# jfkirk/tensorrec

Measured on AMD Instinct MI355X. Metric: user-item predictions/sec, higher is better.
Workload: dtype i8/bf16/fp32; 1 GPU; synthetic 1000000 users x 1000000 items, identity features, d=128, LinearRepresentation + DotProduct, biased, fused top-10 (BASELINE.json configs[2]); users=1000000, items=1000000, n_components=128, top_k=10, parallelism=items sharded x1, users replicated, topk_method=two_stage

## Files before the change

### tensorrec_amd/csrc/score_blockmax_i8.hip

```cpp
#include "score_common.hpp"
#include <math.h>
#include <limits.h>
#include <type_traits>

namespace {

typedef int v4i32 __attribute__((ext_vector_type(4)));
typedef int v16i32 __attribute__((ext_vector_type(16)));

constexpr int BNQ = 128;

template <int KT, bool BIAS, int NCB, int WPS, int TK>
__global__ __launch_bounds__(256, WPS) void blockmax_i8_kernel(ScoreParams p)
{
    constexpr int RB = KT;
    constexpr int CH = RB / 16;
    constexpr int KS = KT / 32;
    constexpr int TILE_BYTES = BNQ * RB;
    constexpr int NSLOT = BNQ * CH / 256;
    constexpr int NBLK = BNQ / 32;
    constexpr int NSTEP = NBLK * KS;
    static_assert(KT == 64 || KT == 128 || KT == 256, "int8 BLOCKMAX covers K = 64 / 128 / 256");

    extern __shared__ __attribute__((aligned(16))) char smem[];
    int* side = (int*)(smem + 2 * TILE_BYTES);

    const int tid = threadIdx.x;
    const int lane = tid & 63;
    const int wave = __builtin_amdgcn_readfirstlane(tid >> 6);
    const int half = lane >> 5, l31 = lane & 31;
    const int rblock = blockIdx.x % p.n_rblocks;
    const int chunk = blockIdx.x / p.n_rblocks;
    const int64_t r_base = ((int64_t)rblock * 4 + wave) * (NCB * 32);
    const int64_t t_begin = (int64_t)chunk * p.chunk_len;
    const int64_t t_end = (t_begin + p.chunk_len < p.n_t) ? t_begin + p.chunk_len : p.n_t;
    const int n_tiles = (int)((t_end - t_begin + BNQ - 1) / BNQ);

    v4i32 rfq[NCB][KS];
    float r_bias[NCB];
#pragma unroll
    for (int cb = 0; cb < NCB; ++cb) {
        int64_t row = r_base + cb * 32 + l31;
        if (row >= p.n_r) row = p.n_r - 1;
        const char* src = (const char*)p.R + row * (int64_t)RB;
#pragma unroll
        for (int ks = 0; ks < KS; ++ks) rfq[cb][ks] = *(const v4i32*)(src + (ks * 2 + half) * 16);
        r_bias[cb] = (BIAS && p.r_bias) ? p.r_bias[row] : 0.f;
    }

    int slot_off[NSLOT];
#pragma unroll
    for (int i = 0; i < NSLOT; ++i) {
        const int q = i * 256 + tid;
        const int row = q / CH, pc = q % CH;
        const int sw = CH >= 16 ? (row & 15) : (CH == 8 ? ((row >> 1) & 7) : ((row >> 2) & 3));
        slot_off[i] = row * RB + ((pc ^ sw) * 16);
    }
    const char* t_chunk = (const char*)p.T + t_begin * (int64_t)RB;
    const int* t_bias_q = p.t_bias ? (const int*)p.t_bias + (p.wg_class ? (int64_t)p.wg_class[rblock] * p.bias_stride : 0) : nullptr;
    auto stage_issue = [&](int tile, int buf) {
        const int64_t row0 = t_begin + (int64_t)tile * BNQ;
        const bool clamp = row0 + BNQ > p.n_t;
        if (BIAS && wave < 2) {
            int64_t g = row0 + wave * 64 + lane;
            if (g >= p.n_t) g = p.n_t - 1;
            if (t_bias_q) {
                __builtin_amdgcn_global_load_lds((const __attribute__((address_space(1))) void*)(t_bias_q + g),
                                                 (__attribute__((address_space(3))) void*)(side + buf * BNQ + wave * 64), 4, 0, 0);
            } else {
                side[buf * BNQ + wave * 64 + lane] = 0;
            }
        }
        const char* tile_base = t_chunk + (int64_t)tile * (BNQ * RB);
#pragma unroll
        for (int i = 0; i < NSLOT; ++i) {
            int off = slot_off[i];
            if (clamp) {
                const int last = (int)(p.n_t - 1 - row0);
                const int row = (i * 256 + tid) / CH;
                if (row > last) off -= (row - last) * RB;
            }
            char* dst = smem + buf * TILE_BYTES + (i * 256 + wave * 64) * 16;
            __builtin_amdgcn_global_load_lds((const __attribute__((address_space(1))) void*)(tile_base + off),
                                             (__attribute__((address_space(3))) void*)dst, 16, 0, 0);
        }
    };

    int koff[KS];
    {
        const int sw = CH >= 16 ? (l31 & 15) : (CH == 8 ? ((l31 >> 1) & 7) : ((l31 >> 2) & 3));
#pragma unroll
        for (int ks = 0; ks < KS; ++ks) koff[ks] = l31 * RB + (((ks * 2 + half) ^ sw) * 16);
    }

    v16i32 acc[NCB];
    int bm[NCB];
#pragma unroll
    for (int cb = 0; cb < NCB; ++cb) bm[cb] = INT_MIN;
    float top[TK ? NCB : 1][TK ? TK : 1];
    float e_nx[TK ? NCB : 1], e_ex[TK ? NCB : 1], e_cu[TK ? NCB : 1];
    if (TK) {
#pragma unroll
        for (int cb = 0; cb < NCB; ++cb) {
            int64_t row = r_base + cb * 32 + l31;
            if (row >= p.n_r) row = p.n_r - 1;
            e_nx[cb] = p.r_err[row * 4]; e_ex[cb] = p.r_err[row * 4 + 1]; e_cu[cb] = p.r_err[row * 4 + 2];
#pragma unroll
            for (int j = 0; j < TK; ++j) top[cb][j] = -INFINITY;
        }
    }

    auto read_c0 = [&](v16i32& c, const int* sdi) {
#pragma unroll
        for (int q = 0; q < 4; ++q) {
            const v4i32 tb4 = *(const v4i32*)(sdi + 8 * q);
            c[4 * q] = tb4[0]; c[4 * q + 1] = tb4[1]; c[4 * q + 2] = tb4[2]; c[4 * q + 3] = tb4[3];
        }
    };

    auto tile_body = [&](auto bufc) __attribute__((always_inline)) {
        constexpr int buf = decltype(bufc)::value;
        const char* tb = smem + buf * TILE_BYTES;
        const int* sd = side + buf * BNQ + 4 * half;
        v4i32 tf[3];
        if (BIAS) read_c0(acc[0], sd);
        tf[0] = *(const v4i32*)(tb + koff[0]);
        tf[1] = *(const v4i32*)(tb + (KS > 1 ? koff[1 % KS] : 32 * RB + koff[0]));
        __builtin_amdgcn_sched_barrier(0);
#pragma unroll
        for (int s = 0; s < NSTEP; ++s) {
            const int blk = s / KS, ks = s % KS;
            if (s + 2 < NSTEP)
                tf[(s + 2) % 3] = *(const v4i32*)(tb + ((s + 2) / KS) * 32 * RB + koff[(s + 2) % KS]);
            if (ks == 0) {
                if (BIAS) {
#pragma unroll
                    for (int cb = NCB - 1; cb >= 0; --cb)
                        acc[cb] = __builtin_amdgcn_mfma_i32_32x32x32_i8(tf[s % 3], rfq[cb][0], acc[0], 0, 0, 0);
                } else {
                    const v16i32 z = {0, 0, 0, 0, 0, 0, 0, 0, 0, 0, 0, 0, 0, 0, 0, 0};
#pragma unroll
                    for (int cb = 0; cb < NCB; ++cb)
                        acc[cb] = __builtin_amdgcn_mfma_i32_32x32x32_i8(tf[s % 3], rfq[cb][0], z, 0, 0, 0);
                }
            } else {
#pragma unroll
                for (int cb = 0; cb < NCB; ++cb)
                    acc[cb] = __builtin_amdgcn_mfma_i32_32x32x32_i8(tf[s % 3], rfq[cb][ks], acc[cb], 0, 0, 0);
            }
            if (ks == KS - 1) {
#pragma unroll
                for (int j = 0; j < 8; ++j) bm[0] = max(max(bm[0], acc[0][2 * j]), acc[0][2 * j + 1]);
                if (BIAS && blk + 1 < NBLK) read_c0(acc[0], sd + 32 * (blk + 1));
#pragma unroll
                for (int j = 0; j < 8; ++j)
#pragma unroll
                    for (int cb = 1; cb < NCB; ++cb) bm[cb] = max(max(bm[cb], acc[cb][2 * j]), acc[cb][2 * j + 1]);
            }
            __builtin_amdgcn_sched_barrier(0);
        }
    };

    stage_issue(0, 0);
    asm volatile("s_waitcnt vmcnt(0)" ::: "memory");
    __syncthreads();

    const float a_user = p.wg_scale ? p.wg_scale[rblock] : p.scales[0];
    const int64_t sb0 = t_begin / ((int64_t)p.sb_tiles * BNQ);
    f32x4 ss_cur = *(const f32x4*)(p.sb_stats + sb0 * 4), ss_next = ss_cur;
    for (int t = 0; t < n_tiles; ++t) {
        const int buf = t & 1;
        if (t + 1 < n_tiles) stage_issue(t + 1, buf ^ 1);
        if ((t % p.sb_tiles) == 0 && t + p.sb_tiles < n_tiles)
            ss_next = *(const f32x4*)(p.sb_stats + (sb0 + t / p.sb_tiles + 1) * 4);
        if (buf == 0) tile_body(std::integral_constant<int, 0>{});
        else tile_body(std::integral_constant<int, 1>{});

        if (((t + 1) % p.sb_tiles) == 0 || t + 1 == n_tiles) {
            const int64_t sb = sb0 + t / p.sb_tiles;
            const float scale = a_user * ss_cur[0];
            const float yh = TK ? ss_cur[1] : 0.f, dy = TK ? ss_cur[2] : 0.f, db = TK ? a_user * ss_cur[3] : 0.f;
            ss_cur = ss_next;
#pragma unroll
            for (int cb = 0; cb < NCB; ++cb) {
                const int o = __shfl_xor(bm[cb], 32, 64);
                const int m = bm[cb] > o ? bm[cb] : o;
                float v = (float)m * scale;
                if (BIAS) v = v + r_bias[cb];
                const int64_t u = r_base + cb * 32 + l31;
                if (half == 0 && u < p.n_r) p.blockmax[sb * p.bm_stride + u] = v;
                bm[cb] = INT_MIN;
                if (TK) {
                    float lb = v - i8_pair_err(e_nx[cb], e_ex[cb], e_cu[cb], yh, dy, db, KT);
                    lb = (lb == lb) ? lb : -INFINITY;
                    if (p.top_tag) lb = lb_tag(lb, t / p.sb_tiles);
#pragma unroll
                    for (int j = TK - 1; j >= 1; --j) top[cb][j] = __builtin_amdgcn_fmed3f(top[cb][j], top[cb][j - 1], lb);
                    top[cb][0] = fmaxf(top[cb][0], lb);
                }
            }
        }
        if (t + 1 < n_tiles) asm volatile("s_waitcnt vmcnt(0)" ::: "memory");
        __syncthreads();
    }
    if (TK) {
#pragma unroll
        for (int cb = 0; cb < NCB; ++cb) {
            const int64_t u = r_base + cb * 32 + l31;
            if (half == 0 && u < p.n_r) {
#pragma unroll
                for (int j = 0; j < TK; ++j) p.chunk_top[((int64_t)chunk * TK + j) * p.bm_stride + u] = top[cb][j];
            }
        }
    }
}

template <int KT, bool BIAS, int TK, int NUB, int NW, int BT, int RDL = 1>
__global__ __launch_bounds__(NW * 64, 8 / NW) void blockmax_i8x16_kernel(ScoreParams p)
{
    constexpr int NT = NW * 64;
    constexpr int OW = NUB / 4;
    static_assert(NUB % 4 == 0, "user blocks per wave must split over the four row-groups");
    constexpr int RB = KT;
    constexpr int CH = RB / 16;
    constexpr int KS = KT / 64;
    constexpr int TILE_BYTES = BT * RB;
    constexpr int NSLOT = BT * CH / NT;
    constexpr int NBLK = BT / 16;
    constexpr int NSTEP = NBLK * KS;
    static_assert(KT == 64 || KT == 128, "int8 16x16x64 BLOCKMAX covers K = 64 / 128");

    extern __shared__ __attribute__((aligned(16))) char smem[];
    int* side = (int*)(smem + 2 * TILE_BYTES);

    const int tid = threadIdx.x;
    const int lane = tid & 63;
    const int wave = __builtin_amdgcn_readfirstlane(tid >> 6);
    const int g = lane >> 4, lu = lane & 15;
    const int rblock = blockIdx.x % p.n_rblocks;
    const int chunk = blockIdx.x / p.n_rblocks;
    if (p.wg_scale && p.wg_scale[rblock] == 0.f) return;
    const int64_t r_base = ((int64_t)rblock * NW + wave) * (NUB * 16);
    const int64_t t_begin = (int64_t)chunk * p.chunk_len;
    const int64_t t_end = (t_begin + p.chunk_len < p.n_t) ? t_begin + p.chunk_len : p.n_t;
    const int n_tiles = (int)((t_end - t_begin + BT - 1) / BT);
    auto swz = [](int row) { return CH == 8 ? (row & 7) : ((row >> 1) & 3); };

    v4i32 rfq[NUB][KS];
#pragma unroll
    for (int ub = 0; ub < NUB; ++ub) {
        int64_t row = r_base + ub * 16 + lu;
        if (row >= p.n_r) row = p.n_r - 1;
        const char* src = (const char*)p.R + row * (int64_t)RB;
#pragma unroll
        for (int ks = 0; ks < KS; ++ks) rfq[ub][ks] = *(const v4i32*)(src + (ks * 4 + g) * 16);
    }
    int64_t own_u[OW];
    float own_bias[OW], e_nx[OW], e_ex[OW], e_cu[OW];
    float top[TK ? OW : 1][TK ? TK : 1];
#pragma unroll
    for (int o = 0; o < OW; ++o) {
        own_u[o] = r_base + (OW * g + o) * 16 + lu;
        const int64_t row = own_u[o] < p.n_r ? own_u[o] : p.n_r - 1;
        own_bias[o] = (BIAS && p.r_bias) ? p.r_bias[row] : 0.f;
        if (TK) {
            e_nx[o] = p.r_err[row * 4]; e_ex[o] = p.r_err[row * 4 + 1]; e_cu[o] = p.r_err[row * 4 + 2];
#pragma unroll
            for (int j = 0; j < TK; ++j) top[o][j] = -INFINITY;
        }
    }

    int slot_off[NSLOT];
#pragma unroll
    for (int i = 0; i < NSLOT; ++i) {
        const int q = i * NT + tid;
        const int row = q / CH, pc = q % CH;
        slot_off[i] = row * RB + ((pc ^ swz(row)) * 16);
    }
    const char* t_chunk = (const char*)p.T + t_begin * (int64_t)RB;
    const int* t_bias_q = p.t_bias ? (const int*)p.t_bias + (p.wg_class ? (int64_t)p.wg_class[rblock] * p.bias_stride : 0) : nullptr;
    auto stage_issue = [&](int tile, int buf) {
        const int64_t row0 = t_begin + (int64_t)tile * BT;
        const bool clamp = row0 + BT > p.n_t;
        if (BIAS && wave < BT / 64) {
            int64_t gi = row0 + wave * 64 + lane;
            if (gi >= p.n_t) gi = p.n_t - 1;
            if (t_bias_q) {
                __builtin_amdgcn_global_load_lds((const __attribute__((address_space(1))) void*)(t_bias_q + gi),
                                                 (__attribute__((address_space(3))) void*)(side + buf * BT + wave * 64), 4, 0, 0);
            } else {
                side[buf * BT + wave * 64 + lane] = 0;
            }
        }
        const char* tile_base = t_chunk + (int64_t)tile * (BT * RB);
#pragma unroll
        for (int i = 0; i < NSLOT; ++i) {
            int off = slot_off[i];
            if (clamp) {
                const int last = (int)(p.n_t - 1 - row0);
                const int row = (i * NT + tid) / CH;
                if (row > last) off -= (row - last) * RB;
            }
            char* dst = smem + buf * TILE_BYTES + (i * NT + wave * 64) * 16;
            __builtin_amdgcn_global_load_lds((const __attribute__((address_space(1))) void*)(tile_base + off),
                                             (__attribute__((address_space(3))) void*)dst, 16, 0, 0);
        }
    };

    int koff[KS];
#pragma unroll
    for (int ks = 0; ks < KS; ++ks) koff[ks] = lu * RB + (((ks * 4 + g) ^ swz(lu)) * 16);

    v4i32 acc[NUB];
    int bm[NUB];
#pragma unroll
    for (int ub = 0; ub < NUB; ++ub) bm[ub] = INT_MIN;

    auto tile_body = [&](auto bufc) __attribute__((always_inline)) {
        constexpr int buf = decltype(bufc)::value;
        const char* tb = smem + buf * TILE_BYTES;
        const int* sd = side + buf * BT + 4 * g;
        v4i32 tf[3];
        v4i32 c0 = {0, 0, 0, 0};
        if (BIAS) c0 = *(const v4i32*)sd;
        tf[0] = *(const v4i32*)(tb + koff[0]);
        tf[1] = *(const v4i32*)(tb + (KS > 1 ? koff[1 % KS] : 16 * RB + koff[0]));
        __builtin_amdgcn_sched_barrier(0);
#pragma unroll
        for (int s = 0; s < NSTEP; ++s) {
            const int blk = s / KS, ks = s % KS;
            auto prefetch = [&]() {
                if (s + 2 < NSTEP) tf[(s + 2) % 3] = *(const v4i32*)(tb + ((s + 2) / KS) * 16 * RB + koff[(s + 2) % KS]);
            };
            if (RDL == 0) prefetch();
            if (ks == 0) {
#pragma unroll
                for (int ub = 0; ub < NUB; ++ub) {
                    acc[ub] = __builtin_amdgcn_mfma_i32_16x16x64_i8(tf[s % 3], rfq[ub][0], c0, 0, 0, 0);
                    if (RDL == 2 && ub == NUB / 2 - 1) { __builtin_amdgcn_sched_barrier(0); prefetch(); __builtin_amdgcn_sched_barrier(0); }
                }
                if (RDL == 1) __builtin_amdgcn_sched_barrier(0);
                if (BIAS && blk + 1 < NBLK) c0 = *(const v4i32*)(sd + 16 * (blk + 1));
            } else {
#pragma unroll
                for (int ub = 0; ub < NUB; ++ub) {
                    acc[ub] = __builtin_amdgcn_mfma_i32_16x16x64_i8(tf[s % 3], rfq[ub][ks], acc[ub], 0, 0, 0);
                    if (RDL == 2 && ub == NUB / 2 - 1) { __builtin_amdgcn_sched_barrier(0); prefetch(); __builtin_amdgcn_sched_barrier(0); }
                }
                if (RDL == 1) __builtin_amdgcn_sched_barrier(0);
            }
            if (RDL == 1 || RDL == 3) prefetch();
            if (ks == KS - 1) {
#pragma unroll
                for (int ub = 0; ub < NUB; ++ub) {
                    bm[ub] = max(max(bm[ub], acc[ub][0]), acc[ub][1]);
                    bm[ub] = max(max(bm[ub], acc[ub][2]), acc[ub][3]);
                }
            }
            if (RDL == 3) {
                if (ks == KS - 1) {
                    __builtin_amdgcn_sched_group_barrier(0x008, 3, 0);
#pragma unroll
                    for (int i = 0; i < NUB - 3; ++i) {
                        __builtin_amdgcn_sched_group_barrier(0x002, 2, 0);
                        __builtin_amdgcn_sched_group_barrier(0x008, 1, 0);
                        if (i == (NUB - 3) / 2) __builtin_amdgcn_sched_group_barrier(0x100, 1, 0);
                    }
                    __builtin_amdgcn_sched_group_barrier(0x002, 6, 0);
                } else {
                    __builtin_amdgcn_sched_group_barrier(0x008, NUB / 2, 0);
                    __builtin_amdgcn_sched_group_barrier(0x100, 2, 0);
                    __builtin_amdgcn_sched_group_barrier(0x008, NUB - NUB / 2, 0);
                }
            }
            __builtin_amdgcn_sched_barrier(0);
        }
    };

    stage_issue(0, 0);
    asm volatile("s_waitcnt vmcnt(0)" ::: "memory");
    __syncthreads();

    const float a_user = p.wg_scale ? p.wg_scale[rblock] : p.scales[0];
    const int64_t sb0 = t_begin / ((int64_t)p.sb_tiles * BT);
    f32x4 ss_cur = *(const f32x4*)(p.sb_stats + sb0 * 4), ss_next = ss_cur;
    for (int t = 0; t < n_tiles; ++t) {
        const int buf = t & 1;
        if (t + 1 < n_tiles) stage_issue(t + 1, buf ^ 1);
        if ((t % p.sb_tiles) == 0 && t + p.sb_tiles < n_tiles)
            ss_next = *(const f32x4*)(p.sb_stats + (sb0 + t / p.sb_tiles + 1) * 4);
        if (buf == 0) tile_body(std::integral_constant<int, 0>{});
        else tile_body(std::integral_constant<int, 1>{});

        if (((t + 1) % p.sb_tiles) == 0 || t + 1 == n_tiles) {
            const int64_t sb = sb0 + t / p.sb_tiles;
            const float scale = a_user * ss_cur[0];
            const float yh = TK ? ss_cur[1] : 0.f, dy = TK ? ss_cur[2] : 0.f, db = TK ? a_user * ss_cur[3] : 0.f;
            ss_cur = ss_next;
            int m[NUB];
#pragma unroll
            for (int ub = 0; ub < NUB; ++ub) {
                int x = bm[ub];
                const int o1 = __shfl_xor(x, 16, 64);
                x = x > o1 ? x : o1;
                const int o2 = __shfl_xor(x, 32, 64);
                m[ub] = x > o2 ? x : o2;
                bm[ub] = INT_MIN;
            }
#pragma unroll
            for (int o = 0; o < OW; ++o) {
                const int mo = g == 0 ? m[o] : (g == 1 ? m[OW + o] : (g == 2 ? m[2 * OW + o] : m[3 * OW + o]));
                float v = (float)mo * scale;
                if (BIAS) v = v + own_bias[o];
                if (own_u[o] < p.n_r) p.blockmax[sb * p.bm_stride + own_u[o]] = v;
                if (TK) {
                    float lb = v - i8_pair_err(e_nx[o], e_ex[o], e_cu[o], yh, dy, db, KT);
                    lb = (lb == lb) ? lb : -INFINITY;
                    if (p.top_tag) lb = lb_tag(lb, t / p.sb_tiles);
#pragma unroll
                    for (int j = TK - 1; j >= 1; --j) top[o][j] = __builtin_amdgcn_fmed3f(top[o][j], top[o][j - 1], lb);
                    top[o][0] = fmaxf(top[o][0], lb);
                }
            }
        }
        if (t + 1 < n_tiles) asm volatile("s_waitcnt vmcnt(0)" ::: "memory");
        __syncthreads();
    }
    if (TK) {
#pragma unroll
        for (int o = 0; o < OW; ++o)
            if (own_u[o] < p.n_r) {
#pragma unroll
                for (int j = 0; j < TK; ++j) p.chunk_top[((int64_t)chunk * TK + j) * p.bm_stride + own_u[o]] = top[o][j];
            }
    }
}

template <int KT, bool BIAS, int TK, int NUB, int NW, int BT, int RDL = 1>
int launch_i8x16(ScoreParams p, int sb_rows, hipStream_t st)
{
    constexpr int LDS = 2 * BT * KT + 2 * BT * 4;
    auto kern = blockmax_i8x16_kernel<KT, BIAS, TK, NUB, NW, BT, RDL>;
    static bool attr_set = false;
    if (!attr_set && LDS > 32 * 1024) {
        (void)hipFuncSetAttribute((const void*)kern, hipFuncAttributeMaxDynamicSharedMemorySize, LDS);
        attr_set = true;
    }
    p.n_rblocks = (int)ceil_div64(p.n_r, NW * NUB * 16);
    p.sb_tiles = sb_rows / BT;
    const unsigned blocks = (unsigned)p.n_rblocks * (unsigned)p.n_chunks;
    hipLaunchKernelGGL(kern, dim3(blocks), dim3(NW * 64), LDS, st, p);
    return trec_check_launch("trec_score_gemm_blockmax_i8 (16x16x64)");
}

template <int KT, bool BIAS, int NCB, int WPS, int TK>
int launch_i8(ScoreParams p, int sb_rows, hipStream_t st)
{
    constexpr int LDS = 2 * BNQ * KT + 2 * BNQ * 4;
    auto kern = blockmax_i8_kernel<KT, BIAS, NCB, WPS, TK>;
    static bool attr_set = false;
    if (!attr_set && LDS > 32 * 1024) {
        (void)hipFuncSetAttribute((const void*)kern, hipFuncAttributeMaxDynamicSharedMemorySize, LDS);
        attr_set = true;
    }
    p.n_rblocks = (int)ceil_div64(p.n_r, 4 * NCB * 32);
    p.sb_tiles = sb_rows / BNQ;
    const unsigned blocks = (unsigned)p.n_rblocks * (unsigned)p.n_chunks;
    hipLaunchKernelGGL(kern, dim3(blocks), dim3(256), LDS, st, p);
    return trec_check_launch("trec_score_gemm_blockmax_i8");
}

template <int G>
__global__ __launch_bounds__(256) void prep_i8_kernel(const float* __restrict__ x, int64_t n, int d, int kt,
                                                     const float* __restrict__ scale_ptr, int sb_rows,
                                                     float* __restrict__ sb_stats, signed char* __restrict__ out_q,
                                                     float2* __restrict__ row_stats, int wg_rows)
{
    const int64_t row = ((int64_t)blockIdx.x * blockDim.x + threadIdx.x) / G;
    const bool ok = row < n;
    const int sub = threadIdx.x % G;
    const int64_t sb = sb_rows ? (ok ? row : n - 1) / sb_rows : 0;
    const float scale = sb_rows ? sb_stats[sb * 4] : (wg_rows > 0 ? scale_ptr[(ok ? row : n - 1) / wg_rows] : *scale_ptr);
    const float inv = 1.0f / scale;
    const float* xr = x + (ok ? row : 0) * (int64_t)d;
    float sw = 0.f, se = 0.f;
#pragma unroll
    for (int it = 0; it < 2; ++it) {
        const int c = (it * G + sub) * 4;
        f32x4 v = {0.f, 0.f, 0.f, 0.f};
        if (ok && c < d) {
            if ((d & 3) == 0) v = *(const f32x4*)(xr + c);
            else {
#pragma unroll
                for (int e = 0; e < 4; ++e) if (c + e < d) v[e] = xr[c + e];
            }
        }
        unsigned int pk = 0;
#pragma unroll
        for (int e = 0; e < 4; ++e) {
            float q = rintf(v[e] * inv);
            q = fminf(fmaxf(q, -127.f), 127.f);
            if (!(q == q)) q = 0.f;
            const float err = v[e] - q * scale;
            sw = fmaf(v[e], v[e], sw);
            se = fmaf(err, err, se);
            pk |= ((unsigned int)(int)q & 0xffu) << (8 * e);
        }
        if (ok && c < kt) *(unsigned int*)(out_q + row * (int64_t)kt + c) = pk;
    }
    for (int off = G / 2; off > 0; off >>= 1) { sw += __shfl_xor(sw, off, 64); se += __shfl_xor(se, off, 64); }
    float nw = sqrtf(sw), ne = sqrtf(se);
    if (sub == 0 && ok) row_stats[row] = make_float2(nw, ne);
}

__global__ __launch_bounds__(256) void sb_reduce_kernel(const float2* __restrict__ row_stats, int64_t n, int sb_rows,
                                                       float* __restrict__ sb_stats)
{
    const int64_t s = blockIdx.x;
    const int64_t r0 = s * sb_rows, r1 = (r0 + sb_rows < n) ? r0 + sb_rows : n;
    float g0 = 0.f, g1 = 0.f;
    for (int64_t r = r0 + threadIdx.x; r < r1; r += 256) {
        const float2 st = row_stats[r];
        float a = st.x + st.y, b = st.y;
        if (a != a) a = INFINITY;
        if (b != b) b = INFINITY;
        g0 = fmaxf(g0, a); g1 = fmaxf(g1, b);
    }
    for (int off = 32; off > 0; off >>= 1) { g0 = fmaxf(g0, __shfl_xor(g0, off, 64)); g1 = fmaxf(g1, __shfl_xor(g1, off, 64)); }
    __shared__ float w0[4], w1[4];
    if ((threadIdx.x & 63) == 0) { w0[threadIdx.x >> 6] = g0; w1[threadIdx.x >> 6] = g1; }
    __syncthreads();
    if (threadIdx.x == 0) {
        sb_stats[s * 4 + 1] = fmaxf(fmaxf(w0[0], w0[1]), fmaxf(w0[2], w0[3]));
        sb_stats[s * 4 + 2] = fmaxf(fmaxf(w1[0], w1[1]), fmaxf(w1[2], w1[3]));
    }
}

__global__ __launch_bounds__(1024) void sb_scale_kernel(const float* __restrict__ x, int64_t n, int d, int sb_rows,
                                                       float* __restrict__ sb_stats)
{
    const int64_t s = blockIdx.x;
    const int64_t r0 = s * sb_rows;
    const int64_t r1 = (r0 + sb_rows < n) ? r0 + sb_rows : n;
    const int64_t n_elem = (r1 - r0) * d;
    const float* xs = x + r0 * (int64_t)d;
    float am = 0.f;
    if ((d & 3) == 0) {
        for (int64_t i = (int64_t)threadIdx.x * 4; i < n_elem; i += 4096) {
            const f32x4 v = *(const f32x4*)(xs + i);
#pragma unroll
            for (int e = 0; e < 4; ++e) { const float a = fabsf(v[e]); am = (a > am || a != a) ? a : am; }
        }
    } else {
        for (int64_t i = threadIdx.x; i < n_elem; i += 1024) { const float a = fabsf(xs[i]); am = (a > am || a != a) ? a : am; }
    }
    if (am != am) am = INFINITY;
    for (int off = 32; off > 0; off >>= 1) am = fmaxf(am, __shfl_xor(am, off, 64));
    __shared__ float wmax[16];
    if ((threadIdx.x & 63) == 0) wmax[threadIdx.x >> 6] = am;
    __syncthreads();
    if (threadIdx.x == 0) {
        am = 0.f;
        for (int w = 0; w < 16; ++w) am = fmaxf(am, wmax[w]);
        float sc = am / 127.0f;
        if (!(sc > 0.f) || !(sc < INFINITY)) sc = 1.0f;
        sb_stats[s * 4] = sc;
    }
}

__global__ __launch_bounds__(256) void bias_i8_kernel(const float* __restrict__ bias, int64_t n, const float* __restrict__ ladder,
                                                     const int32_t* __restrict__ class_used, int sb_rows,
                                                     float* __restrict__ sb_stats, int* __restrict__ bias_q,
                                                     float* __restrict__ gstats)
{
    const int64_t s = blockIdx.x;
    const int c = blockIdx.y;
    if (class_used && class_used[c] == 0) return;
    const int64_t r0 = s * sb_rows, r1 = (r0 + sb_rows < n) ? r0 + sb_rows : n;
    const float a_c = ladder[c];
    const float sp = a_c * sb_stats[s * 4];
    int* bq_c = bias_q + (int64_t)c * n;
    float g2 = 0.f, g3 = 0.f;
    for (int64_t i = r0 + threadIdx.x; i < r1; i += 256) {
        const float b = bias[i];
        float bq = rintf(b / sp);
        bq = fminf(fmaxf(bq, -1073741824.f), 1073741824.f);
        if (!(bq == bq)) bq = 0.f;
        bq_c[i] = (int)bq;
        float a2 = fabsf(b), a3 = fabsf(b - bq * sp);
        if (a2 != a2) a2 = INFINITY;
        if (a3 != a3) a3 = INFINITY;
        g2 = fmaxf(g2, a2); g3 = fmaxf(g3, a3);
    }
    for (int off = 32; off > 0; off >>= 1) { g2 = fmaxf(g2, __shfl_xor(g2, off, 64)); g3 = fmaxf(g3, __shfl_xor(g3, off, 64)); }
    __shared__ float w2[4], w3[4];
    if ((threadIdx.x & 63) == 0) { w2[threadIdx.x >> 6] = g2; w3[threadIdx.x >> 6] = g3; }
    __syncthreads();
    if (threadIdx.x == 0) {
        g2 = fmaxf(fmaxf(w2[0], w2[1]), fmaxf(w2[2], w2[3]));
        g3 = fmaxf(fmaxf(w3[0], w3[1]), fmaxf(w3[2], w3[3]));
        float rel = (g3 / a_c) * 1.0000005f;
        if (!(rel == rel)) rel = INFINITY;
        if (__float_as_uint(rel) > *(volatile unsigned int*)(sb_stats + s * 4 + 3))
            atomicMax((unsigned int*)(sb_stats + s * 4 + 3), __float_as_uint(rel));
        if (__float_as_uint(g2) > *(volatile unsigned int*)(gstats + 2)) atomicMax((unsigned int*)(gstats + 2), __float_as_uint(g2));
    }
}

template <int G>
__global__ __launch_bounds__(256) void row_natscale_kernel(const float* __restrict__ x, int64_t n, int d,
                                                          float* __restrict__ nat, float* __restrict__ gmax)
{
    const int64_t row = ((int64_t)blockIdx.x * blockDim.x + threadIdx.x) / G;
    const bool ok = row < n;
    const int sub = threadIdx.x % G;
    const float* xr = x + (ok ? row : 0) * (int64_t)d;
    f32x4 v[2];
    float am = 0.f;
#pragma unroll
    for (int it = 0; it < 2; ++it) {
        const int c = (it * G + sub) * 4;
        v[it] = (f32x4){0.f, 0.f, 0.f, 0.f};
        if (ok && c < d) {
            if ((d & 3) == 0) v[it] = *(const f32x4*)(xr + c);
            else {
#pragma unroll
                for (int e = 0; e < 4; ++e) if (c + e < d) v[it][e] = xr[c + e];
            }
        }
#pragma unroll
        for (int e = 0; e < 4; ++e) { const float a = fabsf(v[it][e]); am = (a > am || a != a) ? a : am; }
    }
    if (am != am) am = INFINITY;
    for (int off = G / 2; off > 0; off >>= 1) am = fmaxf(am, __shfl_xor(am, off, 64));
    float best = am / 127.0f;
    if (am > 0.f && am < INFINITY) {
        float err[3] = {0.f, 0.f, 0.f};
#pragma unroll
        for (int cnd = 0; cnd < 3; ++cnd) {
            const float sc = (am / 127.0f) * (cnd == 0 ? 1.0f : (cnd == 1 ? 0.5f : 0.25f));
            const float inv = 1.0f / sc;
#pragma unroll
            for (int it = 0; it < 2; ++it)
#pragma unroll
                for (int e = 0; e < 4; ++e) {
                    float q = rintf(v[it][e] * inv);
                    q = fminf(fmaxf(q, -127.f), 127.f);
                    const float r = v[it][e] - q * sc;
                    err[cnd] = fmaf(r, r, err[cnd]);
                }
            for (int off = G / 2; off > 0; off >>= 1) err[cnd] += __shfl_xor(err[cnd], off, 64);
        }
        if (err[1] < err[0] && err[1] <= err[2]) best *= 0.5f;
        else if (err[2] < err[0] && err[2] < err[1]) best *= 0.25f;
    }
    if (!(best > 0.f)) best = 0.f;
    if (sub == 0 && ok) nat[row] = best;
    float gm = (sub == 0 && ok) ? best : 0.f;
    for (int off = 32; off > 0; off >>= 1) gm = fmaxf(gm, __shfl_xor(gm, off, 64));
    if ((threadIdx.x & 63) == 0 && __float_as_uint(gm) > *(volatile unsigned int*)gmax) atomicMax((unsigned int*)gmax, __float_as_uint(gm));
}

__global__ __launch_bounds__(256) void user_err_i8_kernel(const float2* __restrict__ ustats, const float* __restrict__ user_bias,
                                                         const float* __restrict__ gstats, int kdim, int64_t n_users,
                                                         const float* __restrict__ scales, const float* __restrict__ wg_scale,
                                                         int wg_rows, float* __restrict__ r_err)
{
    const int64_t u = (int64_t)blockIdx.x * 256 + threadIdx.x;
    if (u >= n_users) return;
    const float2 st = ustats[u];
    const float bu = user_bias ? fabsf(user_bias[u]) : 0.f;
    const float ck = (float)(kdim + 6) * 2.98023224e-07f;
    *(f32x4*)(r_err + u * 4) = (f32x4){st.x, st.y, ck * (bu + gstats[2]), wg_scale ? wg_scale[u / wg_rows] : scales[0]};
}

__global__ __launch_bounds__(256) void sumsq_absmax_kernel(const float* __restrict__ x, int64_t n_elem, double* __restrict__ ws)
{
    double acc = 0.0;
    float am = 0.f;
    for (int64_t i = ((int64_t)blockIdx.x * 256 + threadIdx.x) * 4; i + 3 < n_elem; i += (int64_t)gridDim.x * 1024) {
        const f32x4 v = *(const f32x4*)(x + i);
        acc += (double)v[0] * v[0] + (double)v[1] * v[1] + (double)v[2] * v[2] + (double)v[3] * v[3];
#pragma unroll
        for (int e = 0; e < 4; ++e) { const float a = fabsf(v[e]); am = (a > am || a != a) ? a : am; }
    }
    if (blockIdx.x == 0 && threadIdx.x == 0)
        for (int64_t i = n_elem & ~(int64_t)3; i < n_elem; ++i) {
            acc += (double)x[i] * x[i];
            const float a = fabsf(x[i]);
            am = (a > am || a != a) ? a : am;
        }
    if (am != am) am = INFINITY;
    for (int off = 32; off > 0; off >>= 1) { acc += __shfl_xor(acc, off, 64); am = fmaxf(am, __shfl_xor(am, off, 64)); }
    if ((threadIdx.x & 63) == 0) {
        atomicAdd(ws, acc);
        atomicMax((unsigned int*)(ws + 1), __float_as_uint(am));
    }
}

__global__ void scale_from_stats_kernel(const double* __restrict__ ws, double n_elem, float clip_sigmas, float* __restrict__ scales)
{
    const double rms = sqrt(ws[0] / n_elem);
    const float am = __uint_as_float(*(const unsigned int*)(ws + 1));
    float top = am;
    if (clip_sigmas > 0.f && (float)(clip_sigmas * rms) < top) top = (float)(clip_sigmas * rms);
    float s = top / 127.0f;
    if (!(s > 0.f) || !(s < INFINITY)) s = 1.0f;
    scales[0] = s;
}

}

extern "C" int trec_score_prep_i8(const float* repr, int64_t n, int32_t d, int32_t kpad, int32_t side, float clip_sigmas,
                                  int32_t sb_rows, const float* bias, float* scales, double* workspace, void* out_q,
                                  float* row_stats, int32_t* bias_q, float* sb_stats, float* gstats, void* stream)
{
    TREC_REQUIRE(scales && (side == 0 || side == 1 || side == 2), "trec_score_prep_i8: side must be 0 (users), 1 (items) or 2 (item biases)");
    TREC_REQUIRE(!bias || (bias_q && gstats && side >= 1), "trec_score_prep_i8: a bias needs bias_q, gstats and side 1 / 2");
    TREC_REQUIRE(side == 0 || (sb_stats && sb_rows >= 1), "trec_score_prep_i8: the item side needs sb_stats and sb_rows");
    if (n == 0) return TREC_OK;
    hipStream_t st = (hipStream_t)stream;
    if (side != 2) {
        TREC_REQUIRE(repr && out_q && row_stats, "trec_score_prep_i8: null pointer");
        TREC_REQUIRE(d >= 1 && kpad >= d && kpad % 4 == 0 && kpad <= 128, "trec_score_prep_i8: need d <= kpad <= 128, kpad % 4 == 0");
        TREC_REQUIRE(((uintptr_t)repr % 16) == 0, "trec_score_prep_i8: repr must be 16-byte aligned");
        if (side == 0) {
            TREC_REQUIRE(workspace, "trec_score_prep_i8: the user side needs the 16-byte workspace");
            if (hipMemsetAsync(workspace, 0, 2 * sizeof(double), st) != hipSuccess) {
                trec_set_last_error("trec_score_prep_i8: memset failed");
                return TREC_ERR_LAUNCH;
            }
            const int64_t n_elem = n * (int64_t)d;
            unsigned sb = (unsigned)ceil_div64(n_elem, 1024 * 8);
            if (sb > 4096) sb = 4096;
            if (sb < 1) sb = 1;
            hipLaunchKernelGGL(sumsq_absmax_kernel, dim3(sb), dim3(256), 0, st, repr, n_elem, workspace);
            hipLaunchKernelGGL(scale_from_stats_kernel, dim3(1), dim3(1), 0, st, workspace, (double)n_elem, clip_sigmas, scales);
        } else {
            hipLaunchKernelGGL(sb_scale_kernel, dim3((unsigned)ceil_div64(n, sb_rows)), dim3(1024), 0, st, repr, n, d, sb_rows, sb_stats);
        }
        const int g = kpad >= 128 ? 32 : kpad / 4;
        const unsigned blocks = (unsigned)ceil_div64(n * g, 256);
#define TREC_PQ(GV) hipLaunchKernelGGL(prep_i8_kernel<GV>, dim3(blocks), dim3(256), 0, st, repr, n, d, kpad, scales, side == 1 ? sb_rows : 0, sb_stats, (signed char*)out_q, (float2*)row_stats, 0)
        if (g == 32) TREC_PQ(32);
        else if (g == 16) TREC_PQ(16);
        else TREC_PQ(8);
#undef TREC_PQ
        if (side == 1)
            hipLaunchKernelGGL(sb_reduce_kernel, dim3((unsigned)ceil_div64(n, sb_rows)), dim3(256), 0, st, (const float2*)row_stats, n, sb_rows, sb_stats);
    }
    if (side >= 1 && bias)
        hipLaunchKernelGGL(bias_i8_kernel, dim3((unsigned)ceil_div64(n, sb_rows), 1), dim3(256), 0, st, bias, n, scales, (const int32_t*)nullptr, sb_rows, sb_stats, bias_q, gstats);
    return trec_check_launch("trec_score_prep_i8");
}


extern "C" int trec_score_row_scale_i8(const float* repr, int64_t n, int32_t d, float* nat, float* gmax, void* stream)
{
    TREC_REQUIRE(repr && nat && gmax, "trec_score_row_scale_i8: null pointer");
    TREC_REQUIRE(d >= 1 && d <= 256 && ((uintptr_t)repr % 16) == 0, "trec_score_row_scale_i8: need d <= 256 and 16-byte aligned rows");
    if (n == 0) return TREC_OK;
    const int kp = (d + 3) / 4 * 4;
    const int g = kp > 64 ? 32 : (kp > 32 ? 16 : 8);
    const unsigned blocks = (unsigned)ceil_div64(n * g, 256);
    hipStream_t st = (hipStream_t)stream;
    if (g == 32) hipLaunchKernelGGL(row_natscale_kernel<32>, dim3(blocks), dim3(256), 0, st, repr, n, d, nat, gmax);
    else if (g == 16) hipLaunchKernelGGL(row_natscale_kernel<16>, dim3(blocks), dim3(256), 0, st, repr, n, d, nat, gmax);
    else hipLaunchKernelGGL(row_natscale_kernel<8>, dim3(blocks), dim3(256), 0, st, repr, n, d, nat, gmax);
    return trec_check_launch("trec_score_row_scale_i8");
}

extern "C" int trec_score_prep_i8_users(const float* repr, int64_t n, int32_t d, int32_t kpad, const float* wg_scale,
                                        int32_t wg_rows, void* out_q, float* row_stats, void* stream)
{
    TREC_REQUIRE(repr && wg_scale && out_q && row_stats && wg_rows >= 1, "trec_score_prep_i8_users: bad arguments");
    TREC_REQUIRE(d >= 1 && kpad >= d && kpad % 4 == 0 && kpad <= 128, "trec_score_prep_i8_users: need d <= kpad <= 128, kpad % 4 == 0");
    TREC_REQUIRE(((uintptr_t)repr % 16) == 0, "trec_score_prep_i8_users: repr must be 16-byte aligned");
    if (n == 0) return TREC_OK;
    hipStream_t st = (hipStream_t)stream;
    const int g = kpad >= 128 ? 32 : kpad / 4;
    const unsigned blocks = (unsigned)ceil_div64(n * g, 256);
#define TREC_PQU(GV) hipLaunchKernelGGL(prep_i8_kernel<GV>, dim3(blocks), dim3(256), 0, st, repr, n, d, kpad, wg_scale, 0, (float*)nullptr, (signed char*)out_q, (float2*)row_stats, wg_rows)
    if (g == 32) TREC_PQU(32);
    else if (g == 16) TREC_PQU(16);
    else TREC_PQU(8);
#undef TREC_PQU
    return trec_check_launch("trec_score_prep_i8_users");
}

extern "C" int trec_score_bias_i8_classes(const float* bias, int64_t n, int32_t sb_rows, const float* ladder,
                                          const int32_t* class_used, int32_t n_classes, float* sb_stats, int32_t* bias_q,
                                          float* gstats, void* stream)
{
    TREC_REQUIRE(bias && ladder && sb_stats && bias_q && gstats, "trec_score_bias_i8_classes: null pointer");
    TREC_REQUIRE(sb_rows >= 1 && n_classes >= 1 && n_classes <= 65535, "trec_score_bias_i8_classes: bad sizes");
    if (n == 0) return TREC_OK;
    hipLaunchKernelGGL(bias_i8_kernel, dim3((unsigned)ceil_div64(n, sb_rows), (unsigned)n_classes), dim3(256), 0, (hipStream_t)stream,
                       bias, n, ladder, class_used, sb_rows, sb_stats, bias_q, gstats);
    return trec_check_launch("trec_score_bias_i8_classes");
}

extern "C" int32_t trec_score_blockmax_i8_rows_per_workgroup(int32_t top_k)
{
    if (trec_get_tuning("blockmax_i8_mfma", 1) == 0) return 4 * 4 * 32;
    const int waves = trec_get_tuning("blockmax_i8_waves", 4) == 8 ? 8 : 4;
    const int users = trec_get_tuning("blockmax_i8_users", top_k > 10 ? 128 : 192) == 192 ? 192 : 128;
    return waves * users;
}

extern "C" int trec_score_user_err_i8(const float* user_stats, const float* user_bias, const float* gstats, int32_t kdim,
                                      int64_t n_users, const float* scales, const float* wg_scale, int32_t wg_rows,
                                      float* r_err, void* stream)
{
    TREC_REQUIRE(user_stats && gstats && r_err && kdim >= 1, "trec_score_user_err_i8: bad arguments");
    TREC_REQUIRE((wg_scale && wg_rows >= 1) || scales, "trec_score_user_err_i8: need wg_scale + wg_rows or scales");
    TREC_REQUIRE(((uintptr_t)r_err % 16) == 0, "trec_score_user_err_i8: r_err must be 16-byte aligned");
    if (n_users == 0) return TREC_OK;
    hipLaunchKernelGGL(user_err_i8_kernel, dim3((unsigned)ceil_div64(n_users, 256)), dim3(256), 0, (hipStream_t)stream,
                       (const float2*)user_stats, user_bias, gstats, kdim, n_users, scales, wg_scale, wg_rows, r_err);
    return trec_check_launch("trec_score_user_err_i8");
}

extern "C" int trec_score_gemm_blockmax_i8(const void* users_q, const void* items_q, int32_t kpad, int64_t n_users,
                                           int64_t n_items, const float* user_bias, const int32_t* item_bias_q,
                                           const float* scales, const float* sb_stats, int32_t sb_rows, int32_t n_chunks,
                                           float* blockmax, int64_t bm_stride, const float* user_err, float* chunk_top,
                                           int32_t top_k, const float* wg_scale, const int32_t* wg_class, int32_t wg_rows,
                                           void* stream)
{
    const int top_tag = (top_k & 0x100) ? 1 : 0;
    top_k &= 0xff;
    TREC_REQUIRE(!wg_scale || wg_rows == trec_score_blockmax_i8_rows_per_workgroup(top_k ? top_k : 10),
                 "trec_score_gemm_blockmax_i8: the user operand was laid out for another workgroup height (tuning changed since the preparation?)");
    TREC_REQUIRE(users_q && items_q && (scales || wg_scale) && sb_stats && blockmax && bm_stride >= n_users, "trec_score_gemm_blockmax_i8: bad arguments");
    TREC_REQUIRE(!wg_class || wg_scale, "trec_score_gemm_blockmax_i8: wg_class comes with wg_scale");
    TREC_REQUIRE(kpad == 64 || kpad == 128, "trec_score_gemm_blockmax_i8: kpad must be 64 or 128");
    TREC_REQUIRE(sb_rows >= BNQ && sb_rows % BNQ == 0, "trec_score_gemm_blockmax_i8: sb_rows must be a multiple of 128");
    TREC_REQUIRE(n_users >= 1 && n_items >= 1 && n_chunks >= 1, "trec_score_gemm_blockmax_i8: empty operand");
    TREC_REQUIRE(n_items < (int64_t)1 << 31 && n_users < (int64_t)1 << 31, "trec_score_gemm_blockmax_i8: sizes must fit int32");
    TREC_REQUIRE((chunk_top != nullptr) == (user_err != nullptr) && (chunk_top ? (top_k == 10 || top_k == 16) : top_k == 0),
                 "trec_score_gemm_blockmax_i8: user_err, chunk_top and top_k (10 or 16) come together");
    ScoreParams p = {};
    p.R = users_q; p.T = items_q; p.n_r = n_users; p.n_t = n_items;
    p.chunk_len = ceil_div64(ceil_div64(n_items, n_chunks), sb_rows) * sb_rows;
    p.n_chunks = (int)ceil_div64(n_items, p.chunk_len);
    p.r_bias = user_bias; p.t_bias = (const float*)item_bias_q;
    p.blockmax = blockmax; p.bm_stride = bm_stride;
    p.scales = scales; p.sb_stats = sb_stats; p.r_err = user_err; p.chunk_top = chunk_top; p.top_k = top_k;
    p.top_tag = top_tag;
    TREC_REQUIRE(!top_tag || (top_k && p.chunk_len / sb_rows <= (1 << TREC_LB_TAG_BITS)),
                 "trec_score_gemm_blockmax_i8: tagged lower bounds need the lists and chunks of at most 4096 superblocks");
    p.wg_scale = wg_scale; p.wg_class = item_bias_q ? wg_class : nullptr; p.bias_stride = n_items;
    hipStream_t st = (hipStream_t)stream;
    const bool bias = user_bias || item_bias_q;
    if (trec_get_tuning("blockmax_i8_mfma", 1) != 0) {
#define TREC_I8X3(KTV, TKV, NUBV, NWV, BTV) (bias ? launch_i8x16<KTV, true, TKV, NUBV, NWV, BTV>(p, sb_rows, st) : launch_i8x16<KTV, false, TKV, NUBV, NWV, BTV>(p, sb_rows, st))
#define TREC_I8X2(KTV, TKV, NUBV, NWV) (tile == 256 && sb_rows % 256 == 0 ? TREC_I8X3(KTV, TKV, NUBV, NWV, 256) : TREC_I8X3(KTV, TKV, NUBV, NWV, 128))
#define TREC_I8X(KTV, TKV) (users == 192 ? (waves == 8 ? TREC_I8X2(KTV, TKV, 12, 8) : TREC_I8X2(KTV, TKV, 12, 4)) \
                                       : (waves == 8 ? TREC_I8X2(KTV, TKV, 8, 8) : TREC_I8X2(KTV, TKV, 8, 4)))
        const int tile = trec_get_tuning("blockmax_i8_tile", 128);
        const int waves = trec_get_tuning("blockmax_i8_waves", 4);
        const int users = trec_get_tuning("blockmax_i8_users", top_k > 10 ? 128 : 192);
        const int rdl = trec_get_tuning("blockmax_i8_rdlate", 1);
        if (kpad == 128 && top_k == 10 && users == 192 && waves == 4 && tile == 128 && rdl != 1) {
            if (rdl == 2) return bias ? launch_i8x16<128, true, 10, 12, 4, 128, 2>(p, sb_rows, st) : launch_i8x16<128, false, 10, 12, 4, 128, 2>(p, sb_rows, st);
            if (rdl == 3) return bias ? launch_i8x16<128, true, 10, 12, 4, 128, 3>(p, sb_rows, st) : launch_i8x16<128, false, 10, 12, 4, 128, 3>(p, sb_rows, st);
            return bias ? launch_i8x16<128, true, 10, 12, 4, 128, 0>(p, sb_rows, st) : launch_i8x16<128, false, 10, 12, 4, 128, 0>(p, sb_rows, st);
        }
        if (kpad == 128) return top_k == 0 ? TREC_I8X(128, 0) : (top_k == 10 ? TREC_I8X(128, 10) : TREC_I8X(128, 16));
        return top_k == 0 ? TREC_I8X(64, 0) : (top_k == 10 ? TREC_I8X(64, 10) : TREC_I8X(64, 16));
#undef TREC_I8X
#undef TREC_I8X2
#undef TREC_I8X3
    }
#define TREC_I8(KTV, TKV) (bias ? launch_i8<KTV, true, 4, 2, TKV>(p, sb_rows, st) : launch_i8<KTV, false, 4, 2, TKV>(p, sb_rows, st))
    if (kpad == 128) return top_k == 0 ? TREC_I8(128, 0) : (top_k == 10 ? TREC_I8(128, 10) : TREC_I8(128, 16));
    return top_k == 0 ? TREC_I8(64, 0) : (top_k == 10 ? TREC_I8(64, 10) : TREC_I8(64, 16));
#undef TREC_I8
}
```

Measured before the change: 11210 billion predictions/s.

## Use three-buffer LDS ring with counted vmcnt waits in int8 blockmax kernel

Replaces the double-buffered tile staging in the int8 16x16x64 blockmax kernel with a configurable ring of three LDS buffers. It issues two tiles ahead and waits with a counted vmcnt instead of draining all loads each iteration. It also restructures the loop by super-block, using a compile-time super-block size when possible and scalar-address loads for the stats, and simplifies address arithmetic with incrementing pointers. LDS use grows by half a tile set per block, which may reduce occupancy. Optional clock-stamp instrumentation is added behind a compile flag.

```diff
diff --git a/tensorrec_amd/csrc/score_blockmax_i8.hip b/tensorrec_amd/csrc/score_blockmax_i8.hip
--- a/tensorrec_amd/csrc/score_blockmax_i8.hip
+++ b/tensorrec_amd/csrc/score_blockmax_i8.hip
@@ -215,7 +215,19 @@
     }
 }
 
-template <int KT, bool BIAS, int TK, int NUB, int NW, int BT, int RDL = 1>
+#ifdef TREC_I8_DIAG
+constexpr int I8_DIAG_WAVES = 1 << 19;
+__device__ unsigned long long g_i8_clk[(size_t)I8_DIAG_WAVES * 4];
+#define TREC_I8_STAMP() ([]() { __builtin_amdgcn_sched_barrier(0); const unsigned long long c_ = __builtin_amdgcn_s_memtime(); __builtin_amdgcn_sched_barrier(0); return c_; }())
+#endif
+
+template <int N> __device__ __forceinline__ void vm_wait()
+{
+    static_assert(N >= 0 && N < 64, "vmcnt is a 6-bit counter");
+    __builtin_amdgcn_s_waitcnt((N & 15) | ((N >> 4) << 14) | 0x0f70);
+}
+
+template <int KT, bool BIAS, int TK, int NUB, int NW, int BT, int RDL = 1, int RING = 3, int SBT = 0>
 __global__ __launch_bounds__(NW * 64, 8 / NW) void blockmax_i8x16_kernel(ScoreParams p)
 {
     constexpr int NT = NW * 64;
@@ -226,12 +238,16 @@
     constexpr int KS = KT / 64;
     constexpr int TILE_BYTES = BT * RB;
     constexpr int NSLOT = BT * CH / NT;
+    constexpr int SLOT_ROWS = NT / CH;
     constexpr int NBLK = BT / 16;
     constexpr int NSTEP = NBLK * KS;
     static_assert(KT == 64 || KT == 128, "int8 16x16x64 BLOCKMAX covers K = 64 / 128");
+    static_assert(RING >= 2 && RING <= 4, "two to four tile buffers");
+    static_assert(SLOT_ROWS % 8 == 0, "a thread's requests must share one swizzle");
+    static_assert((RING - 2) * (NSLOT + 1) < 64, "the counted wait must fit vmcnt");
 
     extern __shared__ __attribute__((aligned(16))) char smem[];
-    int* side = (int*)(smem + 2 * TILE_BYTES);
+    int* side = (int*)(smem + RING * TILE_BYTES);
 
     const int tid = threadIdx.x;
     const int lane = tid & 63;
@@ -240,10 +256,16 @@
     const int rblock = blockIdx.x % p.n_rblocks;
     const int chunk = blockIdx.x / p.n_rblocks;
     if (p.wg_scale && p.wg_scale[rblock] == 0.f) return;
+#ifdef TREC_I8_DIAG
+    const unsigned long long dg_t0 = TREC_I8_STAMP();
+    unsigned long long dg_a = 0, dg_b = 0, dg_c = 0, dg_rel = 0;
+#endif
     const int64_t r_base = ((int64_t)rblock * NW + wave) * (NUB * 16);
     const int64_t t_begin = (int64_t)chunk * p.chunk_len;
     const int64_t t_end = (t_begin + p.chunk_len < p.n_t) ? t_begin + p.chunk_len : p.n_t;
     const int n_tiles = (int)((t_end - t_begin + BT - 1) / BT);
+    const int last_rows = (int)(t_end - t_begin) - (n_tiles - 1) * BT;
+    const int n_plain = last_rows < BT ? n_tiles - 1 : n_tiles;
     auto swz = [](int row) { return CH == 8 ? (row & 7) : ((row >> 1) & 3); };
 
     v4i32 rfq[NUB][KS];
@@ -255,13 +277,14 @@
 #pragma unroll
         for (int ks = 0; ks < KS; ++ks) rfq[ub][ks] = *(const v4i32*)(src + (ks * 4 + g) * 16);
     }
-    int64_t own_u[OW];
+    const int own_l = OW * g * 16 + lu;
+    const int own_n = (int)((p.n_r - r_base < NUB * 16) ? (p.n_r - r_base > 0 ? p.n_r - r_base : 0) : NUB * 16);
     float own_bias[OW], e_nx[OW], e_ex[OW], e_cu[OW];
     float top[TK ? OW : 1][TK ? TK : 1];
 #pragma unroll
     for (int o = 0; o < OW; ++o) {
-        own_u[o] = r_base + (OW * g + o) * 16 + lu;
-        const int64_t row = own_u[o] < p.n_r ? own_u[o] : p.n_r - 1;
+        const int64_t u = r_base + own_l + 16 * o;
+        const int64_t row = u < p.n_r ? u : p.n_r - 1;
         own_bias[o] = (BIAS && p.r_bias) ? p.r_bias[row] : 0.f;
         if (TK) {
             e_nx[o] = p.r_err[row * 4]; e_ex[o] = p.r_err[row * 4 + 1]; e_cu[o] = p.r_err[row * 4 + 2];
@@ -270,41 +293,52 @@
         }
     }
 
-    int slot_off[NSLOT];
-#pragma unroll
-    for (int i = 0; i < NSLOT; ++i) {
-        const int q = i * NT + tid;
-        const int row = q / CH, pc = q % CH;
-        slot_off[i] = row * RB + ((pc ^ swz(row)) * 16);
-    }
-    const char* t_chunk = (const char*)p.T + t_begin * (int64_t)RB;
+    const unsigned slot0 = (unsigned)((tid / CH) * RB + (((tid % CH) ^ swz(tid / CH)) * 16));
     const int* t_bias_q = p.t_bias ? (const int*)p.t_bias + (p.wg_class ? (int64_t)p.wg_class[rblock] * p.bias_stride : 0) : nullptr;
-    auto stage_issue = [&](int tile, int buf) {
-        const int64_t row0 = t_begin + (int64_t)tile * BT;
-        const bool clamp = row0 + BT > p.n_t;
+    const bool bias_dma = BIAS && t_bias_q != nullptr && wave < BT / 64;
+    const char* src_tile = (const char*)p.T + t_begin * (int64_t)RB;
+    const int* src_bias = t_bias_q ? t_bias_q + t_begin + wave * 64 : nullptr;
+    int t_req = 0, buf_req = 0;
+    auto stage_issue = [&](auto clampc) __attribute__((always_inline)) {
+        constexpr bool CLAMPED = decltype(clampc)::value;
+        char* dst = smem + buf_req * TILE_BYTES;
+#pragma unroll
+        for (int i = 0; i < NSLOT; ++i) {
+            const char* src = src_tile + i * (SLOT_ROWS * RB) + slot0;
+            if (CLAMPED) {
+                const int row = i * SLOT_ROWS + tid / CH;
+                if (row > last_rows - 1) src -= (row - (last_rows - 1)) * RB;
+            }
+            __builtin_amdgcn_global_load_lds((const __attribute__((address_space(1))) void*)src,
+                                             (__attribute__((address_space(3))) void*)(dst + (i * NT + wave * 64) * 16), 16, 0, 0);
+        }
         if (BIAS && wave < BT / 64) {
-            int64_t gi = row0 + wave * 64 + lane;
-            if (gi >= p.n_t) gi = p.n_t - 1;
             if (t_bias_q) {
-                __builtin_amdgcn_global_load_lds((const __attribute__((address_space(1))) void*)(t_bias_q + gi),
-                                                 (__attribute__((address_space(3))) void*)(side + buf * BT + wave * 64), 4, 0, 0);
+                int bl = lane;
+                if (CLAMPED && wave * 64 + lane > last_rows - 1) bl = last_rows - 1 - wave * 64;
+                __builtin_amdgcn_global_load_lds((const __attribute__((address_space(1))) void*)(src_bias + bl),
+                                                 (__attribute__((address_space(3))) void*)(side + buf_req * BT + wave * 64), 4, 0, 0);
             } else {
-                side[buf * BT + wave * 64 + lane] = 0;
-            }
-        }
-        const char* tile_base = t_chunk + (int64_t)tile * (BT * RB);
-#pragma unroll
-        for (int i = 0; i < NSLOT; ++i) {
-            int off = slot_off[i];
-            if (clamp) {
-                const int last = (int)(p.n_t - 1 - row0);
-                const int row = (i * NT + tid) / CH;
-                if (row > last) off -= (row - last) * RB;
-            }
-            char* dst = smem + buf * TILE_BYTES + (i * NT + wave * 64) * 16;
-            __builtin_amdgcn_global_load_lds((const __attribute__((address_space(1))) void*)(tile_base + off),
-                                             (__attribute__((address_space(3))) void*)dst, 16, 0, 0);
-        }
+                side[buf_req * BT + wave * 64 + lane] = 0;
+            }
+        }
+        src_tile += TILE_BYTES;
+        if (BIAS) src_bias += BT;
+        ++t_req;
+        buf_req = buf_req + 1 == RING ? 0 : buf_req + 1;
+    };
+    auto request_next = [&]() __attribute__((always_inline)) {
+        if (t_req < n_plain) stage_issue(std::false_type{});
+        else if (t_req < n_tiles) stage_issue(std::true_type{});
+    };
+    auto wait_all_but = [&](int k) __attribute__((always_inline)) {
+        if (RING == 2 || k <= 0) vm_wait<0>();
+        else if (RING == 3 || k == 1) { if (bias_dma) vm_wait<NSLOT + 1>(); else vm_wait<NSLOT>(); }
+        else { if (bias_dma) vm_wait<(RING > 3 ? 2 : 1) * (NSLOT + 1)>(); else vm_wait<(RING > 3 ? 2 : 1) * NSLOT>(); }
+    };
+    auto lds_barrier = [&]() __attribute__((always_inline)) {
+        asm volatile("s_waitcnt lgkmcnt(0)" ::: "memory");
+        __builtin_amdgcn_s_barrier();
     };
 
     int koff[KS];
@@ -326,6 +360,10 @@
         tf[0] = *(const v4i32*)(tb + koff[0]);
         tf[1] = *(const v4i32*)(tb + (KS > 1 ? koff[1 % KS] : 16 * RB + koff[0]));
         __builtin_amdgcn_sched_barrier(0);
+#ifdef TREC_I8_DIAG
+        asm volatile("s_waitcnt lgkmcnt(0)" ::: "memory");
+        dg_c += TREC_I8_STAMP() - dg_rel;
+#endif
 #pragma unroll
         for (int s = 0; s < NSTEP; ++s) {
             const int blk = s / KS, ks = s % KS;
@@ -377,74 +415,117 @@
         }
     };
 
-    stage_issue(0, 0);
-    asm volatile("s_waitcnt vmcnt(0)" ::: "memory");
-    __syncthreads();
-
     const float a_user = p.wg_scale ? p.wg_scale[rblock] : p.scales[0];
-    const int64_t sb0 = t_begin / ((int64_t)p.sb_tiles * BT);
-    f32x4 ss_cur = *(const f32x4*)(p.sb_stats + sb0 * 4), ss_next = ss_cur;
-    for (int t = 0; t < n_tiles; ++t) {
-        const int buf = t & 1;
-        if (t + 1 < n_tiles) stage_issue(t + 1, buf ^ 1);
-        if ((t % p.sb_tiles) == 0 && t + p.sb_tiles < n_tiles)
-            ss_next = *(const f32x4*)(p.sb_stats + (sb0 + t / p.sb_tiles + 1) * 4);
-        if (buf == 0) tile_body(std::integral_constant<int, 0>{});
-        else tile_body(std::integral_constant<int, 1>{});
-
-        if (((t + 1) % p.sb_tiles) == 0 || t + 1 == n_tiles) {
-            const int64_t sb = sb0 + t / p.sb_tiles;
-            const float scale = a_user * ss_cur[0];
-            const float yh = TK ? ss_cur[1] : 0.f, dy = TK ? ss_cur[2] : 0.f, db = TK ? a_user * ss_cur[3] : 0.f;
-            ss_cur = ss_next;
-            int m[NUB];
-#pragma unroll
-            for (int ub = 0; ub < NUB; ++ub) {
-                int x = bm[ub];
-                const int o1 = __shfl_xor(x, 16, 64);
-                x = x > o1 ? x : o1;
-                const int o2 = __shfl_xor(x, 32, 64);
-                m[ub] = x > o2 ? x : o2;
-                bm[ub] = INT_MIN;
-            }
-#pragma unroll
-            for (int o = 0; o < OW; ++o) {
-                const int mo = g == 0 ? m[o] : (g == 1 ? m[OW + o] : (g == 2 ? m[2 * OW + o] : m[3 * OW + o]));
-                float v = (float)mo * scale;
-                if (BIAS) v = v + own_bias[o];
-                if (own_u[o] < p.n_r) p.blockmax[sb * p.bm_stride + own_u[o]] = v;
-                if (TK) {
-                    float lb = v - i8_pair_err(e_nx[o], e_ex[o], e_cu[o], yh, dy, db, KT);
-                    lb = (lb == lb) ? lb : -INFINITY;
-                    if (p.top_tag) lb = lb_tag(lb, t / p.sb_tiles);
-#pragma unroll
-                    for (int j = TK - 1; j >= 1; --j) top[o][j] = __builtin_amdgcn_fmed3f(top[o][j], top[o][j - 1], lb);
-                    top[o][0] = fmaxf(top[o][0], lb);
-                }
-            }
-        }
-        if (t + 1 < n_tiles) asm volatile("s_waitcnt vmcnt(0)" ::: "memory");
-        __syncthreads();
+#pragma unroll
+    for (int i = 0; i < RING - 1; ++i) request_next();
+    wait_all_but(n_tiles - 1 < RING - 2 ? n_tiles - 1 : RING - 2);
+    lds_barrier();
+#ifdef TREC_I8_DIAG
+    dg_rel = TREC_I8_STAMP();
+#endif
+
+    const int sbt = SBT ? SBT : p.sb_tiles;
+    const int64_t sb0 = t_begin / ((int64_t)sbt * BT);
+    const int n_sb = (n_tiles + sbt - 1) / sbt;
+    typedef const __attribute__((address_space(4))) f32x4* sb_stats_ptr;
+    sb_stats_ptr ss_ptr = (sb_stats_ptr)(p.sb_stats + sb0 * 4);
+    float* bm_row = p.blockmax + sb0 * p.bm_stride + r_base;
+    int t = 0, cur = 0;
+    for (int sb = 0; sb < n_sb; ++sb) {
+        const f32x4 ss = *ss_ptr;
+        ++ss_ptr;
+        const int jn = n_tiles - t < sbt ? n_tiles - t : sbt;
+#pragma unroll 1
+        for (int j = 0; j < jn; ++j) {
+            request_next();
+            if (RING == 2) {
+                if (cur == 0) tile_body(std::integral_constant<int, 0>{});
+                else tile_body(std::integral_constant<int, 1>{});
+            } else {
+                if (cur == 0) tile_body(std::integral_constant<int, 0>{});
+                else if (cur == 1) tile_body(std::integral_constant<int, 1>{});
+                else if (RING == 3 || cur == 2) tile_body(std::integral_constant<int, 2>{});
+                else tile_body(std::integral_constant<int, RING - 1>{});
+            }
+            cur = cur + 1 == RING ? 0 : cur + 1;
+            ++t;
+            if (t < n_tiles) {
+#ifdef TREC_I8_DIAG
+                const unsigned long long dg_1 = TREC_I8_STAMP();
+#endif
+                wait_all_but(n_tiles - 1 - t < RING - 2 ? n_tiles - 1 - t : RING - 2);
+#ifdef TREC_I8_DIAG
+                const unsigned long long dg_2 = TREC_I8_STAMP();
+#endif
+                lds_barrier();
+#ifdef TREC_I8_DIAG
+                dg_rel = TREC_I8_STAMP();
+                dg_a += dg_2 - dg_1; dg_b += dg_rel - dg_2;
+#endif
+            }
+        }
+        const float scale = a_user * ss[0];
+        const float yh = TK ? ss[1] : 0.f, dy = TK ? ss[2] : 0.f, db = TK ? a_user * ss[3] : 0.f;
+        int m[NUB];
+#pragma unroll
+        for (int ub = 0; ub < NUB; ++ub) {
+            int x = bm[ub];
+            const int o1 = __shfl_xor(x, 16, 64);
+            x = x > o1 ? x : o1;
+            const int o2 = __shfl_xor(x, 32, 64);
+            m[ub] = x > o2 ? x : o2;
+            bm[ub] = INT_MIN;
+        }
+#pragma unroll
+        for (int o = 0; o < OW; ++o) {
+            const int mo = g == 0 ? m[o] : (g == 1 ? m[OW + o] : (g == 2 ? m[2 * OW + o] : m[3 * OW + o]));
+            float v = (float)mo * scale;
+            if (BIAS) v = v + own_bias[o];
+            if (own_l + 16 * o < own_n) bm_row[own_l + 16 * o] = v;
+            if (TK) {
+                float lb = v - i8_pair_err(e_nx[o], e_ex[o], e_cu[o], yh, dy, db, KT);
+                lb = (lb == lb) ? lb : -INFINITY;
+                if (p.top_tag) lb = lb_tag(lb, sb);
+#pragma unroll
+                for (int j = TK - 1; j >= 1; --j) top[o][j] = __builtin_amdgcn_fmed3f(top[o][j], top[o][j - 1], lb);
+                top[o][0] = fmaxf(top[o][0], lb);
+            }
+        }
+        bm_row += p.bm_stride;
     }
     if (TK) {
 #pragma unroll
         for (int o = 0; o < OW; ++o)
-            if (own_u[o] < p.n_r) {
-#pragma unroll
-                for (int j = 0; j < TK; ++j) p.chunk_top[((int64_t)chunk * TK + j) * p.bm_stride + own_u[o]] = top[o][j];
-            }
-    }
+            if (own_l + 16 * o < own_n) {
+#pragma unroll
+                for (int j = 0; j < TK; ++j) p.chunk_top[((int64_t)chunk * TK + j) * p.bm_stride + r_base + own_l + 16 * o] = top[o][j];
+            }
+    }
+#ifdef TREC_I8_DIAG
+    {
+        const unsigned long long dg_e = TREC_I8_STAMP();
+        const size_t w = (size_t)blockIdx.x * NW + wave;
+        if (lane == 0 && w < (size_t)I8_DIAG_WAVES) {
+            unsigned long long* row = g_i8_clk + w * 4;
+            row[0] = dg_a; row[1] = dg_b; row[2] = dg_c; row[3] = dg_e - dg_t0;
+        }
+    }
+#endif
 }
 
 template <int KT, bool BIAS, int TK, int NUB, int NW, int BT, int RDL = 1>
 int launch_i8x16(ScoreParams p, int sb_rows, hipStream_t st)
 {
-    constexpr int LDS = 2 * BT * KT + 2 * BT * 4;
-    auto kern = blockmax_i8x16_kernel<KT, BIAS, TK, NUB, NW, BT, RDL>;
-    static bool attr_set = false;
-    if (!attr_set && LDS > 32 * 1024) {
+    constexpr int RING = 3;
+    constexpr int LDS = RING * (BT * KT + BT * 4);
+    constexpr bool CONST_SBT = BT == 128 && NW == 4 && RDL == 1;
+    const bool sbt4 = CONST_SBT && sb_rows == 4 * BT;
+    auto kern = sbt4 ? blockmax_i8x16_kernel<KT, BIAS, TK, NUB, NW, BT, RDL, RING, CONST_SBT ? 4 : 0>
+                     : blockmax_i8x16_kernel<KT, BIAS, TK, NUB, NW, BT, RDL, RING, 0>;
+    static bool attr_set[2] = {false, false};
+    if (!attr_set[sbt4] && LDS > 32 * 1024) {
         (void)hipFuncSetAttribute((const void*)kern, hipFuncAttributeMaxDynamicSharedMemorySize, LDS);
-        attr_set = true;
+        attr_set[sbt4] = true;
     }
     p.n_rblocks = (int)ceil_div64(p.n_r, NW * NUB * 16);
     p.sb_tiles = sb_rows / BT;
@@ -878,3 +959,12 @@
     return top_k == 0 ? TREC_I8(64, 0) : (top_k == 10 ? TREC_I8(64, 10) : TREC_I8(64, 16));
 #undef TREC_I8
 }
+
+#ifdef TREC_I8_DIAG
+extern "C" int trec_i8_diag_read(unsigned long long* out, long long n_words)
+{
+    if (n_words > (long long)I8_DIAG_WAVES * 4) n_words = (long long)I8_DIAG_WAVES * 4;
+    if (out && hipMemcpyFromSymbol(out, HIP_SYMBOL(g_i8_clk), sizeof(unsigned long long) * (size_t)n_words) != hipSuccess) return TREC_ERR_LAUNCH;
+    return TREC_OK;
+}
+#endif
```

Result: no change. 11330 billion predictions/s, median of 6 (+1.0%).
